# NVlabs/FoundationPose

Measured on AMD Instinct MI355X. Metric: pose-hypotheses/sec (raster+refine+score), 252 hyp x 160x160 @ 640x480 RGB-D, higher is better.
Workload: dtype f16

## Files before the change

foundationpose_amd/_lib.py:

```python
import ctypes as C
import os

import torch

_HERE = os.path.dirname(os.path.abspath(__file__))
LIB_PATH = os.environ.get("FP_AMD_LIB") or os.path.join(_HERE, "csrc", "libfp_amd.so")
ABI_VERSION = 221
_lib = None

vp, ci, cf, cd, sz = C.c_void_p, C.c_int, C.c_float, C.c_double, C.c_size_t

SIGNATURES = {
    "fp_last_error": (C.c_char_p, []),
    "fp_version": (ci, []),
    "fp_mesh_create": (ci, [vp, vp, vp, vp, vp, vp, vp, ci, ci, ci, ci, C.POINTER(vp)]),
    "fp_mesh_destroy": (None, [vp]),
    "fp_mesh_set_create": (ci, [vp, ci, C.POINTER(vp)]),
    "fp_mesh_set_destroy": (None, [vp]),
    "fp_mesh_set_workspace_bytes": (sz, [vp, ci, ci, ci]),
    "fp_depth_erode": (ci, [vp, vp, ci, ci, ci, cf, cf, cf, vp]),
    "fp_depth_bilateral": (ci, [vp, vp, ci, ci, ci, cf, cf, cf, vp]),
    "fp_depth_to_xyz": (ci, [vp, vp, cf, ci, vp, ci, ci, vp]),
    "fp_crop_windows": (ci, [vp, vp, cd, cd, ci, ci, ci, vp, vp, vp]),
    "fp_crop_windows_multi": (ci, [vp, vp, vp, vp, ci, cd, ci, ci, ci, vp, vp, vp]),
# ... 75 lines not shown
```

foundationpose_amd/csrc/conv_sw.hip:

```cpp
#include <hip/hip_fp16.h>
#include <stdlib.h>
#include <string.h>
#include <type_traits>
#include "igemm_common.h"
#include "igemm_epilogue.h"

#ifdef FP_PROFILE_BUILD
__device__ unsigned long long sw_dbg[8];
extern "C" int fp_dbg_conv_sw(unsigned long long* out, int reset) {
  if (reset) { unsigned long long z[8] = {0, 0, 0, 0, 0, 0, ~0ull, 0}; return (int)hipMemcpyToSymbol(HIP_SYMBOL(sw_dbg), z, sizeof(z)); }
  return (int)hipMemcpyFromSymbol(out, HIP_SYMBOL(sw_dbg), 8 * sizeof(unsigned long long));
}
extern "C" int fp_dbg_conv_sw_epilogue(unsigned long long* out, int reset) {
  if (reset) { unsigned long long z[8] = {0, 0, 0, 0, 0, 0, 0, 0}; return (int)hipMemcpyToSymbol(HIP_SYMBOL(ig_epi_dbg), z, sizeof(z)); }
  return (int)hipMemcpyFromSymbol(out, HIP_SYMBOL(ig_epi_dbg), 8 * sizeof(unsigned long long));
}
#define SW_CLK(t) const unsigned long long t = wall_clock64()
#else
#define SW_CLK(t)
#endif

#ifndef SW_DEFAULT_VARIANT
#define SW_DEFAULT_VARIANT 0
#endif
// ... 5 lines not shown

template <int N>
__device__ __forceinline__ void sw_wait_vm() {
  static_assert(N >= 0 && N < 64, "vmcnt is a 6-bit field");
  asm volatile("s_waitcnt vmcnt(%0)" ::"n"(N) : "memory");
}

__device__ __forceinline__ int sw_q(const IgemmGeom& g, int m) {
  const int b = ig_fastdiv(m, g.mulP, g.shrP);
  const int r = m - b * g.HoWo;
  const int oy = ig_fastdiv(r, g.mulW, g.shrW);
  const int ox = r - oy * g.Wo;
  return (b * g.Hp + oy) * g.Wp + ox;
}

template <int BM, int BN, int TM>
__global__ __launch_bounds__(512, 1) void k_conv_sw(IgemmParams p) {
  constexpr int BK = SW_BK, NW = 8, THREADS = 512;
  constexpr int NWN = BN / 64;
  static_assert((BM / (32 * TM)) * NWN == NW, "8 waves");
  constexpr int ROWB = BK * 2;
  constexpr int W_BYTES = BN * ROWB;
  constexpr int SW_PROWS = sw_prows(BM);
  constexpr int SW_PATCH_BYTES = SW_PROWS * ROWB;
  constexpr int WI = BN / 16 / NW;
  constexpr int PI = SW_PROWS / 16 / NW;
  static_assert(WI >= 1 && PI >= 1 && PI <= 7 && SW_PROWS == PI * 16 * NW, "tile shape");
  constexpr int STAGES_BYTES = 2 * SW_PATCH_BYTES + SW_NSTW * W_BYTES;
  constexpr int LDS_MAIN = ig_lds_main<BM, BN>(STAGES_BYTES);
  auto swz = [](int row) { return (row >> 2) & 3; };
  extern __shared__ __attribute__((aligned(16))) unsigned char smem[];
  SW_CLK(t_start);
  unsigned char* const patch = smem;
  unsigned char* const wring = smem + 2 * SW_PATCH_BYTES;
  const int tid = threadIdx.x, lane = tid & 63;
  const int wid = __builtin_amdgcn_readfirstlane(tid >> 6);
  const int grp = wid >> 2;
  const int wm = wid / NWN, wn = wid - wm * NWN;
  float* bias_lds = reinterpret_cast<float*>(smem + LDS_MAIN);

  const int tiles_n = p.N / BN;
  const int nwg = gridDim.x;
  const int xcd = blockIdx.x & 7, loc = blockIdx.x >> 3;
  const int qd8 = nwg >> 3, r8 = nwg & 7;
  const int tile = (xcd < r8 ? xcd * (qd8 + 1) : r8 * (qd8 + 1) + (xcd - r8) * qd8) + loc;
  const int bm = tile / tiles_n, bn = tile - bm * tiles_n;
  const int m0 = bm * BM, n0 = bn * BN;
  const int Cin = p.Cin, Ktot = 9 * Cin, Wp = p.in.Wp;
  const int ncc = Cin / BK;
  ig_bias_to_lds(p, n0, bias_lds, wid, lane);

  const int q0 = sw_q(p.in, m0);
  const int qmax = (p.M / p.in.HoWo) * p.in.Hp * Wp - 1;
  unsigned poff32[PI], woff32[WI];
#pragma unroll
  for (int j = 0; j < PI; ++j) {
    const int row = (wid * PI + j) * 16 + (lane >> 2);
    const int c = (lane & 3) ^ swz(row);
    int q = q0 + row;
    q = q < qmax ? q : qmax;
    poff32[j] = (unsigned)(((long long)q * p.in.cstride + p.in.coff + c * 8) * 2);
  }
#pragma unroll
  for (int j = 0; j < WI; ++j) {
    const int row = (wid * WI + j) * 16 + (lane >> 2);
    const int c = (lane & 3) ^ swz(row);
    woff32[j] = (unsigned)((((size_t)(n0 + row) * Ktot) + c * 8) * 2);
  }
  const bool wpk = (BN == 128) && p.Wpk != nullptr;
  if (wpk) {
#pragma unroll
    for (int j = 0; j < WI; ++j) woff32[j] = (unsigned)(((wid * WI + j) * 64 + lane) * 16);
  }
// ... 3 lines not shown

  auto stage_patch = [&](int cc, int j) {
    unsigned char* dst = patch + (cc & 1) * SW_PATCH_BYTES + (wid * PI + j) * 1024;
    __builtin_amdgcn_raw_ptr_buffer_load_lds(rsA, (__attribute__((address_space(3))) void*)dst, 16, (int)poff32[j],
                                             cc * (BK * 2), 0, 0);
  };
  auto stage_w = [&](int cc, int tap, int slot) {
    const int wsoff = wpk ? wpk_base + (cc * 9 + tap) * W_BYTES : (tap * Cin + cc * BK) * 2;
    unsigned char* dst = wring + slot * W_BYTES + wid * (WI * 1024);
#pragma unroll
    for (int j = 0; j < WI; ++j)
      __builtin_amdgcn_raw_ptr_buffer_load_lds(rsW, (__attribute__((address_space(3))) void*)(dst + j * 1024), 16,
                                               (int)woff32[j], wsoff, 0, 0);
  };

  float16_ acc[2][TM];
#pragma unroll
  for (int i = 0; i < 2; ++i)
#pragma unroll
    for (int j = 0; j < TM; ++j)
#pragma unroll
      for (int e = 0; e < 16; ++e) acc[i][j][e] = 0.f;

  const int frow = lane & 31, fhalf = lane >> 5;
  int arow[TM], w_off[2][2];
#pragma unroll
  for (int t = 0; t < TM; ++t) {
    int m = m0 + wm * (32 * TM) + t * 32 + frow;
    m = m < p.M ? m : p.M - 1;
    arow[t] = sw_q(p.in, m) - q0;
  }
#pragma unroll
  for (int t = 0; t < 2; ++t) {
    const int rw = wn * 64 + t * 32 + frow;
#pragma unroll
    for (int kk = 0; kk < 2; ++kk) w_off[t][kk] = rw * ROWB + (((2 * kk + fhalf) ^ swz(rw)) << 4);
  }

#pragma unroll
  for (int j = 0; j < PI; ++j) stage_patch(0, j);
  stage_w(0, 0, 0);
  stage_w(0, 1, 1);
  stage_w(0, 2, 2);
  sw_wait_vm<2 * WI>();
  __builtin_amdgcn_s_barrier();
  SW_CLK(t_cold);
  if (grp) __builtin_amdgcn_s_barrier();

  half8 fa[2][TM], fw[2][2];
  static_assert(TM == 4, "the four fragment addresses of the next tap are computed behind the four MFMA groups of a k-step");
  int anext[TM];
#pragma unroll
  for (int t = 0; t < TM; ++t) anext[t] = (arow[t] << 6) + ((fhalf ^ swz(arow[t])) << 4);
  auto kstep = [&](int cc, auto tap_c, auto last_c) {
    constexpr int T = decltype(tap_c)::value;
    constexpr bool LAST = decltype(last_c)::value;
    constexpr int ky = T / 3, kx = T - 3 * ky;
    const int s = cc * 9 + T;
    const unsigned char* pb = patch + (cc & 1) * SW_PATCH_BYTES;
    const unsigned char* wb = wring + (s & (SW_NSTW - 1)) * W_BYTES;
    const int shift = ky * Wp + kx;
#pragma unroll
    for (int t = 0; t < TM; ++t) {
      const int a0 = anext[t];
      fa[0][t] = *reinterpret_cast<const half8*>(pb + a0);
      fa[1][t] = *reinterpret_cast<const half8*>(pb + (a0 ^ 32));
    }
    (void)shift;
#pragma unroll
    for (int kk = 0; kk < 2; ++kk)
#pragma unroll
      for (int t = 0; t < 2; ++t) fw[kk][t] = *reinterpret_cast<const half8*>(wb + w_off[t][kk]);
    if constexpr (!LAST) {
      if constexpr (T < PI) stage_patch(cc + 1, T);
      if constexpr (T + 3 < 9) stage_w(cc, T + 3, (s + 3) & (SW_NSTW - 1));
      else stage_w(cc + 1, T - 6, (s + 3) & (SW_NSTW - 1));
      constexpr int NP = (T < PI ? 1 : 0) + ((T >= 1 && T - 1 < PI) ? 1 : 0);
      sw_wait_vm<2 * WI + NP>();
    } else {
      if constexpr (T + 3 < 9) stage_w(cc, T + 3, (s + 3) & (SW_NSTW - 1));
      constexpr int NYOUNGER = T <= 5 ? 2 : (T == 6 ? 1 : 0);
      sw_wait_vm<NYOUNGER * WI>();
    }
    asm volatile("s_waitcnt lgkmcnt(0)" ::: "memory");
    __builtin_amdgcn_sched_barrier(0);
    __builtin_amdgcn_s_barrier();
    __builtin_amdgcn_sched_barrier(0);
    __builtin_amdgcn_s_setprio(1);
    {
      constexpr int TN = (T + 1) % 9, kyn = TN / 3, kxn = TN - 3 * kyn;
      const int shift_n = kyn * Wp + kxn;
#pragma unroll
      for (int kk = 0; kk < 2; ++kk)
#pragma unroll
        for (int i = 0; i < 2; ++i) {
#pragma unroll
          for (int j = 0; j < TM; ++j)
            acc[i][j] = __builtin_amdgcn_mfma_f32_32x32x16_f16(fw[kk][i], fa[kk][j], acc[i][j], 0, 0, 0);
          const int t = kk * 2 + i;
          {
            int ar = arow[t];
            asm volatile("" : "+v"(ar));
            const int pr = ar + shift_n;
            anext[t] = (pr << 6) + ((fhalf ^ swz(pr)) << 4);
          }
        }
    }
    __builtin_amdgcn_s_setprio(0);
    __builtin_amdgcn_sched_barrier(0);
    __builtin_amdgcn_s_barrier();
    __builtin_amdgcn_sched_barrier(0);
  };
  auto chunk = [&](int cc, auto last_c) {
    kstep(cc, std::integral_constant<int, 0>{}, last_c);
    kstep(cc, std::integral_constant<int, 1>{}, last_c);
    kstep(cc, std::integral_constant<int, 2>{}, last_c);
    kstep(cc, std::integral_constant<int, 3>{}, last_c);
    kstep(cc, std::integral_constant<int, 4>{}, last_c);
    kstep(cc, std::integral_constant<int, 5>{}, last_c);
    kstep(cc, std::integral_constant<int, 6>{}, last_c);
    kstep(cc, std::integral_constant<int, 7>{}, last_c);
// ... 181 lines not shown
  ig_epilogue<BM, BN, TM, THREADS, 0>(p, acc, smem, m0, n0, wm, wn, tid, lane, bias_lds);
}

template <int BM, int BN, int TM>
int sw_ls_launch(const IgemmParams& p, hipStream_t stream) {
  constexpr int LDS = 2 * LS_PROWS * SW_BK * 2 + LS_NSTW * BN * SW_BK * 2;
  static_assert(2 * LDS <= 160 * 1024, "two workgroups per CU");
  const long long tiles = (long long)fp_cdiv(p.M, BM) * (p.N / BN);
  FP_REQUIRE(tiles < (1ll << 31), "fp_igemm_f16_fwd: too many tiles");
  FP_SET_MAX_LDS((k_conv_sw_ls<BM, BN, TM>), LDS);
  hipLaunchKernelGGL((k_conv_sw_ls<BM, BN, TM>), dim3((unsigned)tiles), dim3(256), LDS, stream, p);
  FP_CHECK_LAUNCH("fp_igemm_f16_fwd(conv_sw_ls)");
  return FP_OK;
}

template <int BM, int BN, int TM>
int sw_launch(const IgemmParams& p, hipStream_t stream) {
  constexpr int LDS = ig_lds_main<BM, BN>(2 * sw_prows(BM) * SW_BK * 2 + SW_NSTW * BN * SW_BK * 2) + IG_BIAS_LDS;
  static_assert(LDS <= 160 * 1024, "does not fit the 160 KiB LDS");
  const long long tiles = (long long)fp_cdiv(p.M, BM) * (p.N / BN);
  FP_REQUIRE(tiles < (1ll << 31), "fp_igemm_f16_fwd: too many tiles");
  FP_SET_MAX_LDS((k_conv_sw<BM, BN, TM>), LDS);
  hipLaunchKernelGGL((k_conv_sw<BM, BN, TM>), dim3((unsigned)tiles), dim3(512), LDS, stream, p);
  FP_CHECK_LAUNCH("fp_igemm_f16_fwd(conv_sw)");
  return FP_OK;
}

}

static int sw_span(const IgemmGeom& g, int BM) {
  const int row_cross = (BM - 1) / g.Wo + 1, img_cross = (BM - 1) / g.HoWo + 1;
  return (BM - 1) + 2 * row_cross + (2 * g.Wp + 2) * img_cross + 2 * g.Wp + 3;
}

static int sw_variant(const IgemmParams& p) {
  int v = SW_DEFAULT_VARIANT;
#ifdef FP_PROFILE_BUILD
  static int forced = -2;
// ... 19 lines not shown
  const IgemmGeom& g = p.in;
  if (p.taps != 9 || g.stride != 1 || g.off != 0 || g.bsplit != 0) return false;
  if (g.HoWo % g.Wo != 0 || g.Wp != g.Wo + 2 || g.Hp != g.HoWo / g.Wo + 2) return false;
  const int BM = sw_tile_rows(p);
  if (p.M % g.HoWo != 0 || p.M < 2 * BM) return false;
  if (p.Cin % 64 != 0 || p.N % 128 != 0) return false;
  const long long bytes = (long long)(p.M / g.HoWo) * g.Hp * g.Wp * g.cstride * 2;
  if (bytes >= (1ll << 31)) return false;
  return sw_span(g, BM) <= (sw_variant(p) == 1 ? LS_PROWS : sw_prows(BM));
}

int fp_conv3x3_sw_tile_rows(const IgemmParams& p) { return sw_tile_rows(p); }

int fp_conv3x3_sw_launch(const IgemmParams& p, hipStream_t stream) {
  if (sw_variant(p) == 1) return sw_ls_launch<256, 128, 4>(p, stream);
  if (sw_use_256(p)) return sw_launch<256, 256, 4>(p, stream);
  return sw_launch<512, 128, 4>(p, stream);
}

__global__ __launch_bounds__(256) void k_pack_conv3x3_tiles(const _Float16* __restrict__ w, _Float16* __restrict__ out, int N, int Cin) {
  const int nk = 9 * (Cin / 32);
  const long long total = (long long)N * nk * 4;
  const long long q = (long long)blockIdx.x * 256 + threadIdx.x;
  if (q >= total) return;
  const int pc = (int)(q & 3);
  const int r = (int)((q >> 2) & 127);
  const long long blk = q >> 9;
  const int s = (int)(blk % nk), bn = (int)(blk / nk);
  const int cc = s / 9, tap = s - 9 * cc;
  const int lc = pc ^ ((r >> 2) & 3);
  const half8 v = *reinterpret_cast<const half8*>(w + (size_t)(bn * 128 + r) * (9 * Cin) + tap * Cin + cc * 32 + lc * 8);
  *reinterpret_cast<half8*>(out + q * 8) = v;
// ... 13 lines not shown
```

foundationpose_amd/csrc/igemm.hip:

```cpp
#include <hip/hip_fp16.h>
#include <stdlib.h>
#include <string.h>
#include "igemm_common.h"
#include "igemm_epilogue.h"

int fp_igemm_pp_launch(const IgemmParams& p, int variant, hipStream_t stream);
int fp_conv3x3_sw_launch(const IgemmParams& p, hipStream_t stream);
bool fp_conv3x3_sw_applicable(const IgemmParams& p);
int fp_conv3x3_sw_tile_rows(const IgemmParams& p);

template <int BM, int BN, int TM, int NST, int BK, bool SPLITK = false>
__global__ __launch_bounds__((BM / (32 * TM)) * (BN / 64) * 64, ((BM / (32 * TM)) * (BN / 64) == 4 && TM == 4) ? 2 : 1) void k_igemm_f16(IgemmParams p) {
  constexpr int NWN = BN / 64;
  constexpr int NW = (BM / (32 * TM)) * NWN;
  constexpr int THREADS = NW * 64;
  constexpr int ROWB = BK * 2;
  constexpr int CPK = BK / 8;
  constexpr int RPI = 1024 / ROWB;
  constexpr int KK = BK / 16;
  constexpr int A_BYTES = BM * ROWB;
  constexpr int STAGE_BYTES = A_BYTES + BN * ROWB;
  constexpr int AI = BM / RPI / NW;
  constexpr int WI = BN / RPI / NW;
  static_assert(AI >= 1 && WI >= 1, "tile too small for this wave count");
// ... 295 lines not shown
  return ig_launch<128, 128, 2, 2, 64>(p, stream);
}


static int ig_build_params(const void* x, const fp_igemm_geom* x_geom, const void* w, void* y, const fp_igemm_geom* y_geom,
                           int M, int N, int Cin, int taps, const fp_igemm_epilogue* ep, IgemmParams& p, const char* who) {
  FP_REQUIRE(x && w && y && x_geom && y_geom, "%s: NULL tensor / geometry", who);
  FP_REQUIRE(taps == 1 || taps == 9, "%s: taps must be 1 (GEMM) or 9 (3x3 conv), got %d", who, taps);
  FP_REQUIRE(N > 0 && N % 128 == 0, "%s: N=%d must be a multiple of 128", who, N);
  FP_REQUIRE(Cin > 0 && Cin % 64 == 0, "%s: Cin=%d must be a multiple of 64", who, Cin);
  static const fp_igemm_epilogue no_epilogue = {nullptr, nullptr, nullptr, nullptr, nullptr, 0, nullptr, 0, nullptr, nullptr};
  const fp_igemm_epilogue& e = ep ? *ep : no_epilogue;
  FP_REQUIRE(!e.residual || e.r_geom, "%s: residual without geometry", who);
  FP_REQUIRE((e.bn_scale == nullptr) == (e.bn_shift == nullptr), "%s: bn_scale and bn_shift go together", who);
  FP_REQUIRE(!e.bn_scale || (e.flags & FP_IGEMM_ROUND_ACC), "%s: BatchNorm needs FP_IGEMM_ROUND_ACC (conv semantics)", who);
  FP_REQUIRE((e.flags & ~(FP_IGEMM_RELU | FP_IGEMM_ROUND_ACC | FP_IGEMM_HAS_W_TILES)) == 0, "%s: unknown flags 0x%x", who, e.flags);
  FP_REQUIRE((e.pe == nullptr) == (e.y_pe == nullptr) && (!e.pe || e.pe_period > 0), "%s: pe, pe_period and y_pe go together", who);
  FP_REQUIRE((((size_t)x | (size_t)w | (size_t)y | (size_t)e.residual | (size_t)e.bias | (size_t)e.bn_scale | (size_t)e.bn_shift |
               (size_t)e.pe | (size_t)e.y_pe) & 15) == 0, "%s: tensors must be 16-byte aligned", who);
  if (int err = ig_check_geom(x_geom, "input", who)) return err;
  if (int err = ig_check_geom(y_geom, "output", who)) return err;
  if (e.residual) if (int err = ig_check_geom(e.r_geom, "residual", who)) return err;
  const void* w_tiles = (e.flags & FP_IGEMM_HAS_W_TILES) ? e.w_tiles : nullptr;
  FP_REQUIRE(!w_tiles || (taps == 9 && (((size_t)w_tiles) & 15) == 0 && w_tiles != w), "%s: w_tiles is for 3x3 convolutions, 16-byte aligned, not w itself", who);
  p.A = (const _Float16*)x; p.Wt = (const _Float16*)w; p.Wpk = (const _Float16*)w_tiles; p.bias = e.bias; p.bn_scale = e.bn_scale; p.bn_shift = e.bn_shift;
  p.R = (const _Float16*)e.residual; p.Y = (_Float16*)y;
  p.pe = e.pe; p.Ype = (_Float16*)e.y_pe; p.pe_period = e.pe_period;
  p.M = M; p.N = N; p.Cin = Cin; p.taps = taps; p.relu = (e.flags & FP_IGEMM_RELU) ? 1 : 0;
  p.round_acc = (e.flags & FP_IGEMM_ROUND_ACC) ? 1 : 0;
  p.in = ig_geom(x_geom); p.out = ig_geom(y_geom); p.res = e.residual ? ig_geom(e.r_geom) : ig_geom(y_geom);
  p.slab = nullptr; p.nsplit = 0;
  return FP_OK;
}

extern "C" int fp_igemm_f16_fwd(const void* x, const fp_igemm_geom* x_geom, const void* w, void* y, const fp_igemm_geom* y_geom,
                                int M, int N, int Cin, int taps, const fp_igemm_epilogue* ep, void* stream) {
  FP_REQUIRE(M >= 0, "fp_igemm_f16_fwd: M < 0");
  if (M == 0) return FP_OK;
  IgemmParams p;
  if (int err = ig_build_params(x, x_geom, w, y, y_geom, M, N, Cin, taps, ep, p, "fp_igemm_f16_fwd")) return err;
  return ig_dispatch(p, (hipStream_t)stream);
}

extern "C" size_t fp_igemm_splitk_workspace_bytes(int M, int N, int splits) {
// ... 23 lines not shown
```

foundationpose_amd/csrc/igemm_common.h:

```cpp
#pragma once
#include <hip/hip_fp16.h>
#include "fp_common.h"

typedef _Float16 half8 __attribute__((ext_vector_type(8)));
typedef _Float16 half4 __attribute__((ext_vector_type(4)));
typedef float float16_ __attribute__((ext_vector_type(16)));

#define IG_BK 64

struct IgemmGeom {
  int HoWo, Wo;
  int Hp, Wp;
  int stride;
  int off;
  int cstride;
  int coff;
  int bsplit;
  int cgroup;
  unsigned mulP, shrP;
  unsigned mulW, shrW;
  unsigned mulB, shrB;
};

static inline void ig_fastdiv_init(int d, unsigned* mul, unsigned* shr) {
// ... 12 lines not shown
  const _Float16* A;
  const _Float16* Wt;
  const _Float16* Wpk;
  const float* bias;
  const float* bn_scale;
  const float* bn_shift;
  const _Float16* R;
  _Float16* Y;
  const float* pe;
  _Float16* Ype;
  int pe_period;
  int M, N, Cin, taps;
  int relu;
  int round_acc;
  IgemmGeom in, out, res;
  float* slab;
  int nsplit;
};

__device__ __forceinline__ long long ig_row_off(const IgemmGeom& g, int m) {
  const int b = ig_fastdiv(m, g.mulP, g.shrP);
  const int r = m - b * g.HoWo;
  const int oy = ig_fastdiv(r, g.mulW, g.shrW);
  const int ox = r - oy * g.Wo;
  int bb = b, cg = 0;
  if (g.bsplit > 0) { cg = ig_fastdiv(b, g.mulB, g.shrB); bb = b - cg * g.bsplit; }
  return (((long long)bb * g.Hp + (oy * g.stride + g.off)) * g.Wp + (ox * g.stride + g.off)) * g.cstride + g.coff +
         (long long)cg * g.cgroup;
}

// ... 1 lines not shown
```

foundationpose_amd/csrc/igemm_epilogue.h:

```cpp
#pragma once
#include "igemm_common.h"

#ifdef FP_PROFILE_BUILD
static __device__ unsigned long long ig_epi_dbg[8];
#define IG_CLK(t) const unsigned long long t = wall_clock64()
#else
#define IG_CLK(t)
#endif

#define IG_VEC_FLOATS 256
#define IG_BIAS_LDS (3 * IG_VEC_FLOATS * 4)

template <int BM, int BN>
constexpr int ig_lds_main(int stage_bytes) {
  return stage_bytes > BM * BN * 2 + BM * 16 ? stage_bytes : BM * BN * 2 + BM * 16;
}

template <int BM, int BN, int TM, int THREADS, int DBG, bool FULL>
__device__ __forceinline__ void ig_epilogue_body(const IgemmParams& p, float16_ (&acc)[2][TM], unsigned char* smem, int m0, int n0,
                                                 int wm, int wn, int tid, int lane, const float* bias_lds) {
  constexpr int CPR = BN / 8;
  constexpr int NIT = (BM * CPR) / THREADS;
  unsigned char* E = smem;
  typedef float float4_ __attribute__((ext_vector_type(4)));
  const bool round_acc = p.round_acc != 0, has_bn = p.bn_scale != nullptr;
  long long* rowY = reinterpret_cast<long long*>(smem + BM * 2 * BN);
  long long* rowR = rowY + BM;
  IG_CLK(te0);
  for (int r = tid; r < BM; r += THREADS) {
    const int m = m0 + r;
    const bool in = m < p.M;
    rowY[r] = in ? ig_row_off(p.out, m) + n0 : -1;
    if (p.R) rowR[r] = in ? ig_row_off(p.res, m) + n0 : 0;
  }
  __syncthreads();
  IG_CLK(te1);
  half8 rv[NIT];
  if (p.R) {
#pragma unroll
    for (int it = 0; it < NIT; ++it) {
      const int qd = tid + it * THREADS;
      const int ml = qd / CPR, ch = qd % CPR;
      if (FULL || rowY[ml] >= 0) rv[it] = *reinterpret_cast<const half8*>(p.R + rowR[ml] + ch * 8);
    }
  }
  IG_CLK(te2);
#pragma unroll
  for (int i = 0; i < 2; ++i) {
#pragma unroll
    for (int g = 0; g < 4; ++g) {
      const int nl = wn * 64 + i * 32 + 8 * g + 4 * (lane >> 5);
      const float4_ bv = *reinterpret_cast<const float4_*>(bias_lds + nl);
      float4_ sc = {1.f, 1.f, 1.f, 1.f}, sh = {0.f, 0.f, 0.f, 0.f};
      if (has_bn) {
        sc = *reinterpret_cast<const float4_*>(bias_lds + IG_VEC_FLOATS + nl);
        sh = *reinterpret_cast<const float4_*>(bias_lds + 2 * IG_VEC_FLOATS + nl);
      }
#pragma unroll
      for (int j = 0; j < TM; ++j) {
        const int ml = wm * (32 * TM) + j * 32 + (lane & 31);
        half4 v;
        if (round_acc) {
          typedef _Float16 half2_ __attribute__((ext_vector_type(2)));
          const half2_ b01 = {(_Float16)bv[0], (_Float16)bv[1]}, b23 = {(_Float16)bv[2], (_Float16)bv[3]};
          half2_ t01 = {(_Float16)acc[i][j][g * 4 + 0], (_Float16)acc[i][j][g * 4 + 1]};
          half2_ t23 = {(_Float16)acc[i][j][g * 4 + 2], (_Float16)acc[i][j][g * 4 + 3]};
          t01 = t01 + b01;
          t23 = t23 + b23;
          if (has_bn) {
            v[0] = (_Float16)fmaf((float)t01[0], sc[0], sh[0]);
            v[1] = (_Float16)fmaf((float)t01[1], sc[1], sh[1]);
            v[2] = (_Float16)fmaf((float)t23[0], sc[2], sh[2]);
            v[3] = (_Float16)fmaf((float)t23[1], sc[3], sh[3]);
          } else {
            v[0] = t01[0]; v[1] = t01[1]; v[2] = t23[0]; v[3] = t23[1];
          }
        } else {
#pragma unroll
          for (int e = 0; e < 4; ++e) v[e] = (_Float16)(acc[i][j][g * 4 + e] + bv[e]);
        }
        const int chunk = (nl >> 3) ^ (ml & 15);
        *reinterpret_cast<half4*>(E + ml * (2 * BN) + (chunk << 4) + ((nl & 4) << 1)) = v;
      }
    }
  }
  __syncthreads();
  IG_CLK(te3);
  const half8 zero = {0, 0, 0, 0, 0, 0, 0, 0};
#pragma unroll
  for (int it = 0; it < NIT; ++it) {
    const int qd = tid + it * THREADS;
    const int ml = qd / CPR, ch = qd % CPR;
    const long long yo = rowY[ml];
    if (!FULL && yo < 0) continue;
    half8 v = *reinterpret_cast<const half8*>(E + ml * (2 * BN) + ((ch ^ (ml & 15)) << 4));
    if (p.R) v = v + rv[it];
    if (p.relu) v = __builtin_elementwise_max(v, zero);
// ... 5 lines not shown
      half8 w;
#pragma unroll
      for (int e = 0; e < 4; ++e) { w[e] = (_Float16)((float)v[e] + e0[e]); w[4 + e] = (_Float16)((float)v[4 + e] + e1[e]); }
      *reinterpret_cast<half8*>(p.Ype + (size_t)m * p.N + n0 + ch * 8) = w;
    }
  }
#ifdef FP_PROFILE_BUILD
  IG_CLK(te4);
  if (tid == 0) {
    atomicAdd(&ig_epi_dbg[0], te1 - te0); atomicAdd(&ig_epi_dbg[1], te2 - te1); atomicAdd(&ig_epi_dbg[2], te3 - te2);
    atomicAdd(&ig_epi_dbg[3], te4 - te3); atomicAdd(&ig_epi_dbg[4], 1ull);
  }
#endif
}

template <int BM, int BN, int TM, int THREADS, int DBG = 0>
__device__ __forceinline__ void ig_epilogue(const IgemmParams& p, float16_ (&acc)[2][TM], unsigned char* smem, int m0, int n0,
                                            int wm, int wn, int tid, int lane, const float* bias_lds) {
  if (m0 + BM <= p.M) ig_epilogue_body<BM, BN, TM, THREADS, DBG, true>(p, acc, smem, m0, n0, wm, wn, tid, lane, bias_lds);
  else ig_epilogue_body<BM, BN, TM, THREADS, DBG, false>(p, acc, smem, m0, n0, wm, wn, tid, lane, bias_lds);
}
__device__ __forceinline__ void ig_bias_to_lds(const IgemmParams& p, int n0, float* bias_lds, int wid, int lane) {
  if (wid > 2) return;
  const float* src = wid == 0 ? p.bias : (wid == 1 ? p.bn_scale : p.bn_shift);
  float* dst = bias_lds + wid * IG_VEC_FLOATS;
  if (src) {
    const __amdgpu_buffer_rsrc_t rs = __builtin_amdgcn_make_buffer_rsrc(const_cast<float*>(src), 0, p.N * 4, 0x00020000);
    __builtin_amdgcn_raw_ptr_buffer_load_lds(rs, (__attribute__((address_space(3))) void*)dst, 16, lane * 16, n0 * 4, 0, 0);
  } else if (wid == 0) {
    typedef float f4 __attribute__((ext_vector_type(4)));
    *reinterpret_cast<f4*>(dst + lane * 4) = f4{0.f, 0.f, 0.f, 0.f};
  }
// ... 2 lines not shown
```

foundationpose_amd/engine.py:

```python
import contextlib

import torch
import torch.nn.functional as F

from . import ops

USE_MIOPEN = False


FUSED_OUT_PROJ_LN = True


FUSED_FFN = True


ROWS_QKV = True
ROWS_QKV_MIN_ROWS = 4096
PACKED_CONV_TILES = True
MERGED_HEAD_QKV = True
FUSED_TAIL = True


def _conv_backend():
    if USE_MIOPEN or not torch.backends.cudnn.is_available():
        return contextlib.nullcontext()
    return torch.backends.cudnn.flags(enabled=False)


def _bn_affine(sd, bn_p):
    if bn_p is None or (bn_p + ".weight") not in sd:
        return None, None
    scale = sd[bn_p + ".weight"].float() / torch.sqrt(sd[bn_p + ".running_var"].float() + 1e-5)
    shift = sd[bn_p + ".bias"].float() - sd[bn_p + ".running_mean"].float() * scale
    return scale.contiguous(), shift.contiguous()

# ... 92 lines not shown
    w = sd[conv_p + ".weight"].float()
    b = sd.get(conv_p + ".bias")
    scale, shift = _bn_affine(sd, bn_p)
    wk = w.permute(0, 2, 3, 1).reshape(w.shape[0], -1).to(torch.float16).contiguous()
    tiles = None
    if wk.is_cuda and w.shape[2] == 3 and w.shape[3] == 3 and w.shape[0] % 128 == 0 and w.shape[1] % 32 == 0 and PACKED_CONV_TILES:
        tiles = ops.pack_conv3x3_tiles(wk, w.shape[0], w.shape[1])
    return dict(w=wk, w_tiles=tiles, bias=None if b is None else _r16(b.float()), scale=scale, shift=shift)


SPLITK_MAX_HYPS = 12
HEADS_TWO_STREAMS_MAX_HYPS = 12
SPLITK_TARGET_WGS = 384
SMALL_CALL_CEILING = 31

_SWITCHES = ("FUSED_OUT_PROJ_LN", "FUSED_FFN", "ROWS_QKV", "PACKED_CONV_TILES", "MERGED_HEAD_QKV", "FUSED_TAIL", "SPLITK_MAX_HYPS", "HEADS_TWO_STREAMS_MAX_HYPS")


@contextlib.contextmanager
def overrides(**kw):
    g = globals()
    for k, v in kw.items():
        if k not in _SWITCHES:
            raise KeyError(f"engine.overrides: unknown switch {k!r} (known: {', '.join(_SWITCHES)})")
        if k.endswith("_MAX_HYPS") and not (0 <= int(v) <= SMALL_CALL_CEILING):
            raise ValueError(f"engine.overrides: {k} = {v} is outside 0..{SMALL_CALL_CEILING}")
    saved = {k: g[k] for k in kw}
    g.update(kw)
    try:
        yield
    finally:
# ... 375 lines not shown
```

foundationpose_amd/ops.py:

```python
import ctypes as C
from typing import NamedTuple

import numpy as np
import torch

from . import _lib

FLAG_NORMALIZE_XYZ = 1
FLAG_OUT_F16 = 2
MODE_REFINE = 0
MODE_SCORE = 1
ROT_AXIS_ANGLE = 0
ROT_6D = 1
TRANS_TRACKNET, TRANS_DEEPIM, TRANS_RAW = 0, 1, 2


def _stream(t=None):
    if t is None:
        return C.c_void_p(torch.cuda.current_stream().cuda_stream)
    dev = t.device
    if dev.index is not None and dev.index != torch.cuda.current_device():
        raise _lib.FpAmdError(f"tensor on {dev} but the current device is cuda:{torch.cuda.current_device()}: wrap the call in "
                              f"`with torch.cuda.device({dev.index}):` (kernels launch on the current device)")
    return C.c_void_p(torch.cuda.current_stream(dev).cuda_stream)
# ... 911 lines not shown
                                       "coff", "bsplit", "cgroup")]

    @staticmethod
    def matrix(ld):
        return IgemmGeom(1, 1, 1, 1, 1, 0, int(ld), 0, 0, 0)

    @staticmethod
    def image(Ho, Wo, pad, C_, stride=1, offset=None, coff=0, bsplit=0, cgroup=0):
        return IgemmGeom(Ho * Wo, Wo, Ho * stride + 2 * pad, Wo * stride + 2 * pad, stride, pad if offset is None else offset,
                         C_, coff, bsplit, cgroup)


IGEMM_RELU = 1
IGEMM_ROUND_ACC = 2
IGEMM_HAS_W_TILES = 4


class IgemmEpilogue(C.Structure):
    _fields_ = [("bias", C.c_void_p), ("bn_scale", C.c_void_p), ("bn_shift", C.c_void_p), ("residual", C.c_void_p),
                ("r_geom", C.POINTER(IgemmGeom)), ("flags", C.c_int), ("pe", C.c_void_p), ("pe_period", C.c_int), ("y_pe", C.c_void_p),
                ("w_tiles", C.c_void_p)]


def pack_conv3x3_tiles(w, N, Cin):
    w = _dev(w, torch.float16, "w")
    out = torch.empty_like(w)
    _lib.check(_lib.lib().fp_pack_conv3x3_tiles_f16(_ptr(w), _ptr(out), int(N), int(Cin), _stream(w)), "fp_pack_conv3x3_tiles_f16")
    return out


def igemm_f16(x, x_geom, w, bias, y, y_geom, M, N, Cin, taps, relu=False, residual=None, r_geom=None, bn_scale=None,
              bn_shift=None, conv_rounding=False, pe=None, y_pe=None, w_tiles=None):
    x = _dev(x, torch.float16, "x"); w = _dev(w, torch.float16, "w"); y = _dev(y, torch.float16, "y")
    b = _dev(bias, torch.float32, "bias"); r = _dev(residual, torch.float16, "residual")
    sc = _dev(bn_scale, torch.float32, "bn_scale"); sh = _dev(bn_shift, torch.float32, "bn_shift")
    pe = _dev(pe, torch.float32, "pe"); y_pe = _dev(y_pe, torch.float16, "y_pe")
    ep = IgemmEpilogue()
    ep.bias, ep.bn_scale, ep.bn_shift = _ptr(b), _ptr(sc), _ptr(sh)
    ep.residual = _ptr(r)
    ep.r_geom = C.pointer(r_geom) if r_geom is not None else None
    ep.flags = (IGEMM_RELU if relu else 0) | (IGEMM_ROUND_ACC if conv_rounding else 0) | IGEMM_HAS_W_TILES
    ep.pe, ep.pe_period, ep.y_pe = _ptr(pe), (int(pe.shape[-2]) if pe is not None else 0), _ptr(y_pe)
    ep.w_tiles = _ptr(_dev(w_tiles, torch.float16, "w_tiles"))
    st = _lib.lib().fp_igemm_f16_fwd(_ptr(x), C.byref(x_geom), _ptr(w), _ptr(y), C.byref(y_geom), int(M), int(N), int(Cin),
                                     int(taps), C.byref(ep), _stream(x))
    _lib.check(st, "fp_igemm_f16_fwd")
    return y


def igemm_splitk_workspace_bytes(M, N, splits):
    return int(_lib.lib().fp_igemm_splitk_workspace_bytes(int(M), int(N), int(splits)))


def igemm_f16_splitk(x, x_geom, w, bias, y, y_geom, M, N, Cin, taps, splits, workspace, relu=False, residual=None, r_geom=None,
                     bn_scale=None, bn_shift=None, conv_rounding=False, pe=None, y_pe=None):
    x = _dev(x, torch.float16, "x"); w = _dev(w, torch.float16, "w"); y = _dev(y, torch.float16, "y")
# ... 439 lines not shown
```

include/fp_amd.h:

```cpp
#ifndef FP_AMD_H
#define FP_AMD_H

#include <stddef.h>
#include <stdint.h>

#ifdef __cplusplus
extern "C" {
#endif

typedef enum {
  FP_OK = 0,
  FP_ERR_INVALID_ARG = -1,
  FP_ERR_WORKSPACE = -2,
  FP_ERR_LAUNCH = -3,
  FP_ERR_UNSUPPORTED = -4
} fp_status;

#define FP_FLAG_NORMALIZE_XYZ 1
#define FP_FLAG_OUT_F16 2

#define FP_MODE_REFINE 0
#define FP_MODE_SCORE 1

#define FP_ROT_AXIS_ANGLE 0
#define FP_ROT_6D 1
#define FP_TRANS_TRACKNET 0
#define FP_TRANS_DEEPIM 1
#define FP_TRANS_RAW 2

#define FP_SUBPIXEL_BITS 4
#define FP_ZBUF_STEPS_PER_METRE 1048576
#define FP_ZBUF_EMPTY 0xFFFFFFFFu

typedef struct fp_mesh fp_mesh;
typedef struct fp_mesh_set fp_mesh_set;

const char* fp_last_error(void);
#define FP_AMD_ABI_VERSION 221
int fp_version(void);

int fp_mesh_create(const float* pos , const float* nrm , const int32_t* faces ,
                   const float* uv , const int32_t* uv_idx ,
                   const float* tex , const float* vcol , int V, int T, int Ht,
                   int Wt, fp_mesh** out);
void fp_mesh_destroy(fp_mesh* mesh);

#define FP_MESH_SET_MAX_ELEMS (1 << 26)
int fp_mesh_set_create(const fp_mesh* const* meshes , int M, fp_mesh_set** out);
void fp_mesh_set_destroy(fp_mesh_set* set);
size_t fp_mesh_set_workspace_bytes(const fp_mesh_set* set, int N, int oh, int ow);

int fp_depth_erode(const float* depth , float* out , int H, int W, int radius,
                   float depth_diff_thres, float ratio_thres, float zfar, void* stream);
// ... 108 lines not shown
                         float input_w, void* stream);


int fp_conv7x7s2_bn_relu_fwd(const void* x , const void* w , const float* bias ,
                             const float* bn_scale , const float* bn_shift , void* y ,
                             int B, int Hin, int Win, int pad, void* stream);

typedef struct {
  int pixels_per_image, width, padded_h, padded_w, stride, offset, cstride, coff, bsplit, cgroup;
} fp_igemm_geom;

#define FP_IGEMM_RELU 1
#define FP_IGEMM_HAS_W_TILES 4
#define FP_IGEMM_ROUND_ACC 2

typedef struct {
  const float* bias;
  const float* bn_scale;
  const float* bn_shift;
  const void* residual;
  const fp_igemm_geom* r_geom;
  int flags;
  const float* pe;
  int pe_period;
  void* y_pe;
  const void* w_tiles;
} fp_igemm_epilogue;

int fp_igemm_f16_fwd(const void* x , const fp_igemm_geom* x_geom , const void* w , void* y ,
                     const fp_igemm_geom* y_geom , int M, int N, int Cin, int taps,
// ... 74 lines not shown
```

Baseline: 7489.

## Add 16x16x32 MFMA variant of the sliding-window 3x3 conv kernel

Adds a templated S16 path to the sliding-window conv kernel that uses 16x16x32 f16 MFMA instructions instead of 32x32x16. This changes fragment layout, LDS swizzle, accumulator shape and the epilogue mapping. It is selected by a new igemm flag and enabled by default from Python. The intent is to use an MFMA shape with different latency and throughput and a different LDS access pattern. The cost is more fragment loads and address arithmetic per k-step, and a new swizzle and epilogue layout that must be exactly right.

```diff
diff --git a/foundationpose_amd/_lib.py b/foundationpose_amd/_lib.py
--- a/foundationpose_amd/_lib.py
+++ b/foundationpose_amd/_lib.py
@@ -5,7 +5,7 @@
 
 _HERE = os.path.dirname(os.path.abspath(__file__))
 LIB_PATH = os.environ.get("FP_AMD_LIB") or os.path.join(_HERE, "csrc", "libfp_amd.so")
-ABI_VERSION = 221
+ABI_VERSION = 222
 _lib = None
 
 vp, ci, cf, cd, sz = C.c_void_p, C.c_int, C.c_float, C.c_double, C.c_size_t
diff --git a/foundationpose_amd/csrc/conv_sw.hip b/foundationpose_amd/csrc/conv_sw.hip
--- a/foundationpose_amd/csrc/conv_sw.hip
+++ b/foundationpose_amd/csrc/conv_sw.hip
@@ -43,7 +43,7 @@
   return (b * g.Hp + oy) * g.Wp + ox;
 }
 
-template <int BM, int BN, int TM>
+template <int BM, int BN, int TM, bool S16>
 __global__ __launch_bounds__(512, 1) void k_conv_sw(IgemmParams p) {
   constexpr int BK = SW_BK, NW = 8, THREADS = 512;
   constexpr int NWN = BN / 64;
@@ -58,6 +58,7 @@
   constexpr int STAGES_BYTES = 2 * SW_PATCH_BYTES + SW_NSTW * W_BYTES;
   constexpr int LDS_MAIN = ig_lds_main<BM, BN>(STAGES_BYTES);
   auto swz = [](int row) { return (row >> 2) & 3; };
+  auto swzp = [](int row) { return S16 ? (row >> 1) & 2 : (row >> 2) & 3; };
   extern __shared__ __attribute__((aligned(16))) unsigned char smem[];
   SW_CLK(t_start);
   unsigned char* const patch = smem;
@@ -85,7 +86,7 @@
 #pragma unroll
   for (int j = 0; j < PI; ++j) {
     const int row = (wid * PI + j) * 16 + (lane >> 2);
-    const int c = (lane & 3) ^ swz(row);
+    const int c = (lane & 3) ^ swzp(row);
     int q = q0 + row;
     q = q < qmax ? q : qmax;
     poff32[j] = (unsigned)(((long long)q * p.in.cstride + p.in.coff + c * 8) * 2);
@@ -119,27 +120,41 @@
                                                (int)woff32[j], wsoff, 0, 0);
   };
 
-  float16_ acc[2][TM];
-#pragma unroll
-  for (int i = 0; i < 2; ++i)
-#pragma unroll
-    for (int j = 0; j < TM; ++j)
-#pragma unroll
-      for (int e = 0; e < 16; ++e) acc[i][j][e] = 0.f;
-
-  const int frow = lane & 31, fhalf = lane >> 5;
-  int arow[TM], w_off[2][2];
-#pragma unroll
-  for (int t = 0; t < TM; ++t) {
-    int m = m0 + wm * (32 * TM) + t * 32 + frow;
+  constexpr int NFA = S16 ? 2 * TM : TM, NFW = S16 ? 4 : 2;
+  constexpr int FR = S16 ? 16 : 32;
+  typedef float float4_ __attribute__((ext_vector_type(4)));
+  typedef typename std::conditional<S16, float4_, float16_>::type acc_t;
+  acc_t acc[NFW][NFA];
+#pragma unroll
+  for (int i = 0; i < NFW; ++i)
+#pragma unroll
+    for (int j = 0; j < NFA; ++j)
+#pragma unroll
+      for (int e = 0; e < (S16 ? 4 : 16); ++e) acc[i][j][e] = 0.f;
+
+  const int frow = lane & (FR - 1), fhalf = lane >> (S16 ? 4 : 5);
+  int arow[NFA], w_off[2][2];
+#pragma unroll
+  for (int t = 0; t < NFA; ++t) {
+    int m = m0 + wm * (32 * TM) + t * FR + frow;
     m = m < p.M ? m : p.M - 1;
     arow[t] = sw_q(p.in, m) - q0;
-  }
-#pragma unroll
-  for (int t = 0; t < 2; ++t) {
-    const int rw = wn * 64 + t * 32 + frow;
-#pragma unroll
-    for (int kk = 0; kk < 2; ++kk) w_off[t][kk] = rw * ROWB + (((2 * kk + fhalf) ^ swz(rw)) << 4);
+    if constexpr (S16) arow[t] = (arow[t] << 6) + (fhalf << 4);
+  }
+  if constexpr (S16) {
+    const int quad = (0x1320 >> (4 * (frow >> 2))) & 3;
+#pragma unroll
+    for (int t = 0; t < 4; ++t) {
+      const int rw = wn * 64 + t * 16 + 4 * quad + (frow & 3);
+      w_off[t >> 1][t & 1] = rw * ROWB + ((fhalf ^ swz(rw)) << 4);
+    }
+  } else {
+#pragma unroll
+    for (int t = 0; t < 2; ++t) {
+      const int rw = wn * 64 + t * 32 + frow;
+#pragma unroll
+      for (int kk = 0; kk < 2; ++kk) w_off[t][kk] = rw * ROWB + (((2 * kk + fhalf) ^ swz(rw)) << 4);
+    }
   }
 
 #pragma unroll
@@ -153,10 +168,11 @@
   if (grp) __builtin_amdgcn_s_barrier();
 
   half8 fa[2][TM], fw[2][2];
-  static_assert(TM == 4, "the four fragment addresses of the next tap are computed behind the four MFMA groups of a k-step");
-  int anext[TM];
-#pragma unroll
-  for (int t = 0; t < TM; ++t) anext[t] = (arow[t] << 6) + ((fhalf ^ swz(arow[t])) << 4);
+  static_assert(TM == 4, "the fragment addresses of the next tap are computed behind the MFMA groups of a k-step, one per group of four");
+  int anext[NFA];
+#pragma unroll
+  for (int t = 0; t < NFA; ++t)
+    anext[t] = S16 ? arow[t] ^ ((arow[t] >> 3) & 32) : (arow[t] << 6) + ((fhalf ^ swz(arow[t])) << 4);
   auto kstep = [&](int cc, auto tap_c, auto last_c) {
     constexpr int T = decltype(tap_c)::value;
     constexpr bool LAST = decltype(last_c)::value;
@@ -165,17 +181,24 @@
     const unsigned char* pb = patch + (cc & 1) * SW_PATCH_BYTES;
     const unsigned char* wb = wring + (s & (SW_NSTW - 1)) * W_BYTES;
     const int shift = ky * Wp + kx;
-#pragma unroll
-    for (int t = 0; t < TM; ++t) {
-      const int a0 = anext[t];
-      fa[0][t] = *reinterpret_cast<const half8*>(pb + a0);
-      fa[1][t] = *reinterpret_cast<const half8*>(pb + (a0 ^ 32));
+    if constexpr (S16) {
+#pragma unroll
+      for (int t = 0; t < NFA; ++t) fa[t >> 2][t & 3] = *reinterpret_cast<const half8*>(pb + anext[t]);
+#pragma unroll
+      for (int t = 0; t < 4; ++t) fw[t >> 1][t & 1] = *reinterpret_cast<const half8*>(wb + w_off[t >> 1][t & 1]);
+    } else {
+#pragma unroll
+      for (int t = 0; t < TM; ++t) {
+        const int a0 = anext[t];
+        fa[0][t] = *reinterpret_cast<const half8*>(pb + a0);
+        fa[1][t] = *reinterpret_cast<const half8*>(pb + (a0 ^ 32));
+      }
+#pragma unroll
+      for (int kk = 0; kk < 2; ++kk)
+#pragma unroll
+        for (int t = 0; t < 2; ++t) fw[kk][t] = *reinterpret_cast<const half8*>(wb + w_off[t][kk]);
     }
     (void)shift;
-#pragma unroll
-    for (int kk = 0; kk < 2; ++kk)
-#pragma unroll
-      for (int t = 0; t < 2; ++t) fw[kk][t] = *reinterpret_cast<const half8*>(wb + w_off[t][kk]);
     if constexpr (!LAST) {
       if constexpr (T < PI) stage_patch(cc + 1, T);
       if constexpr (T + 3 < 9) stage_w(cc, T + 3, (s + 3) & (SW_NSTW - 1));
@@ -195,6 +218,21 @@
     {
       constexpr int TN = (T + 1) % 9, kyn = TN / 3, kxn = TN - 3 * kyn;
       const int shift_n = kyn * Wp + kxn;
+      if constexpr (S16) {
+        int sh = shift_n << 6;
+        asm volatile("" : "+s"(sh));
+#pragma unroll
+        for (int i = 0; i < 4; ++i)
+#pragma unroll
+          for (int jh = 0; jh < 2; ++jh) {
+#pragma unroll
+            for (int j = 0; j < 4; ++j)
+              acc[i][jh * 4 + j] = __builtin_amdgcn_mfma_f32_16x16x32_f16(fw[i >> 1][i & 1], fa[jh][j], acc[i][jh * 4 + j], 0, 0, 0);
+            const int t = i * 2 + jh;
+            const int x = arow[t] + sh;
+            anext[t] = x ^ ((x >> 3) & 32);
+          }
+      } else {
 #pragma unroll
       for (int kk = 0; kk < 2; ++kk)
 #pragma unroll
@@ -210,6 +248,7 @@
             anext[t] = (pr << 6) + ((fhalf ^ swz(pr)) << 4);
           }
         }
+      }
     }
     __builtin_amdgcn_s_setprio(0);
     __builtin_amdgcn_sched_barrier(0);
@@ -421,14 +460,14 @@
   return FP_OK;
 }
 
-template <int BM, int BN, int TM>
+template <int BM, int BN, int TM, bool S16>
 int sw_launch(const IgemmParams& p, hipStream_t stream) {
   constexpr int LDS = ig_lds_main<BM, BN>(2 * sw_prows(BM) * SW_BK * 2 + SW_NSTW * BN * SW_BK * 2) + IG_BIAS_LDS;
   static_assert(LDS <= 160 * 1024, "does not fit the 160 KiB LDS");
   const long long tiles = (long long)fp_cdiv(p.M, BM) * (p.N / BN);
   FP_REQUIRE(tiles < (1ll << 31), "fp_igemm_f16_fwd: too many tiles");
-  FP_SET_MAX_LDS((k_conv_sw<BM, BN, TM>), LDS);
-  hipLaunchKernelGGL((k_conv_sw<BM, BN, TM>), dim3((unsigned)tiles), dim3(512), LDS, stream, p);
+  FP_SET_MAX_LDS((k_conv_sw<BM, BN, TM, S16>), LDS);
+  hipLaunchKernelGGL((k_conv_sw<BM, BN, TM, S16>), dim3((unsigned)tiles), dim3(512), LDS, stream, p);
   FP_CHECK_LAUNCH("fp_igemm_f16_fwd(conv_sw)");
   return FP_OK;
 }
@@ -478,8 +517,8 @@
 
 int fp_conv3x3_sw_launch(const IgemmParams& p, hipStream_t stream) {
   if (sw_variant(p) == 1) return sw_ls_launch<256, 128, 4>(p, stream);
-  if (sw_use_256(p)) return sw_launch<256, 256, 4>(p, stream);
-  return sw_launch<512, 128, 4>(p, stream);
+  if (sw_use_256(p)) return p.mfma16 ? sw_launch<256, 256, 4, true>(p, stream) : sw_launch<256, 256, 4, false>(p, stream);
+  return p.mfma16 ? sw_launch<512, 128, 4, true>(p, stream) : sw_launch<512, 128, 4, false>(p, stream);
 }
 
 __global__ __launch_bounds__(256) void k_pack_conv3x3_tiles(const _Float16* __restrict__ w, _Float16* __restrict__ out, int N, int Cin) {
diff --git a/foundationpose_amd/csrc/igemm.hip b/foundationpose_amd/csrc/igemm.hip
--- a/foundationpose_amd/csrc/igemm.hip
+++ b/foundationpose_amd/csrc/igemm.hip
@@ -333,7 +333,10 @@
   FP_REQUIRE(!e.residual || e.r_geom, "%s: residual without geometry", who);
   FP_REQUIRE((e.bn_scale == nullptr) == (e.bn_shift == nullptr), "%s: bn_scale and bn_shift go together", who);
   FP_REQUIRE(!e.bn_scale || (e.flags & FP_IGEMM_ROUND_ACC), "%s: BatchNorm needs FP_IGEMM_ROUND_ACC (conv semantics)", who);
-  FP_REQUIRE((e.flags & ~(FP_IGEMM_RELU | FP_IGEMM_ROUND_ACC | FP_IGEMM_HAS_W_TILES)) == 0, "%s: unknown flags 0x%x", who, e.flags);
+  FP_REQUIRE((e.flags & ~(FP_IGEMM_RELU | FP_IGEMM_ROUND_ACC | FP_IGEMM_HAS_W_TILES | FP_IGEMM_MFMA_16X16X32 | FP_IGEMM_MFMA_32X32X16)) == 0,
+             "%s: unknown flags 0x%x", who, e.flags);
+  FP_REQUIRE((e.flags & (FP_IGEMM_MFMA_16X16X32 | FP_IGEMM_MFMA_32X32X16)) != (FP_IGEMM_MFMA_16X16X32 | FP_IGEMM_MFMA_32X32X16),
+             "%s: FP_IGEMM_MFMA_16X16X32 and FP_IGEMM_MFMA_32X32X16 exclude each other", who);
   FP_REQUIRE((e.pe == nullptr) == (e.y_pe == nullptr) && (!e.pe || e.pe_period > 0), "%s: pe, pe_period and y_pe go together", who);
   FP_REQUIRE((((size_t)x | (size_t)w | (size_t)y | (size_t)e.residual | (size_t)e.bias | (size_t)e.bn_scale | (size_t)e.bn_shift |
                (size_t)e.pe | (size_t)e.y_pe) & 15) == 0, "%s: tensors must be 16-byte aligned", who);
@@ -347,6 +350,7 @@
   p.pe = e.pe; p.Ype = (_Float16*)e.y_pe; p.pe_period = e.pe_period;
   p.M = M; p.N = N; p.Cin = Cin; p.taps = taps; p.relu = (e.flags & FP_IGEMM_RELU) ? 1 : 0;
   p.round_acc = (e.flags & FP_IGEMM_ROUND_ACC) ? 1 : 0;
+  p.mfma16 = (e.flags & FP_IGEMM_MFMA_32X32X16) ? 0 : ((e.flags & FP_IGEMM_MFMA_16X16X32) ? 1 : SW_DEFAULT_MFMA16);
   p.in = ig_geom(x_geom); p.out = ig_geom(y_geom); p.res = e.residual ? ig_geom(e.r_geom) : ig_geom(y_geom);
   p.slab = nullptr; p.nsplit = 0;
   return FP_OK;
diff --git a/foundationpose_amd/csrc/igemm_common.h b/foundationpose_amd/csrc/igemm_common.h
--- a/foundationpose_amd/csrc/igemm_common.h
+++ b/foundationpose_amd/csrc/igemm_common.h
@@ -7,6 +7,9 @@
 typedef float float16_ __attribute__((ext_vector_type(16)));
 
 #define IG_BK 64
+#ifndef SW_DEFAULT_MFMA16
+#define SW_DEFAULT_MFMA16 1
+#endif
 
 struct IgemmGeom {
   int HoWo, Wo;
@@ -50,6 +53,7 @@
   int relu;
   int round_acc;
   IgemmGeom in, out, res;
+  int mfma16;
   float* slab;
   int nsplit;
 };
diff --git a/foundationpose_amd/csrc/igemm_epilogue.h b/foundationpose_amd/csrc/igemm_epilogue.h
--- a/foundationpose_amd/csrc/igemm_epilogue.h
+++ b/foundationpose_amd/csrc/igemm_epilogue.h
@@ -1,4 +1,5 @@
 #pragma once
+#include <type_traits>
 #include "igemm_common.h"
 
 #ifdef FP_PROFILE_BUILD
@@ -16,9 +17,12 @@
   return stage_bytes > BM * BN * 2 + BM * 16 ? stage_bytes : BM * BN * 2 + BM * 16;
 }
 
-template <int BM, int BN, int TM, int THREADS, int DBG, bool FULL>
-__device__ __forceinline__ void ig_epilogue_body(const IgemmParams& p, float16_ (&acc)[2][TM], unsigned char* smem, int m0, int n0,
+typedef float ig_float4 __attribute__((ext_vector_type(4)));
+template <int BM, int BN, int TM, int THREADS, int DBG, bool FULL, typename Acc>
+__device__ __forceinline__ void ig_epilogue_body(const IgemmParams& p, Acc& acc, unsigned char* smem, int m0, int n0,
                                                  int wm, int wn, int tid, int lane, const float* bias_lds) {
+  constexpr bool S16 = std::is_same<Acc, ig_float4[4][2 * TM]>::value;
+  static_assert(S16 || std::is_same<Acc, float16_[2][TM]>::value, "accumulator layout");
   constexpr int CPR = BN / 8;
   constexpr int NIT = (BM * CPR) / THREADS;
   unsigned char* E = smem;
@@ -45,42 +49,63 @@
     }
   }
   IG_CLK(te2);
+  auto put4 = [&](int nl, int ml, float a0, float a1, float a2, float a3, const float4_& bv, const float4_& sc, const float4_& sh) {
+    half4 v;
+    if (round_acc) {
+      typedef _Float16 half2_ __attribute__((ext_vector_type(2)));
+      const half2_ b01 = {(_Float16)bv[0], (_Float16)bv[1]}, b23 = {(_Float16)bv[2], (_Float16)bv[3]};
+      half2_ t01 = {(_Float16)a0, (_Float16)a1};
+      half2_ t23 = {(_Float16)a2, (_Float16)a3};
+      t01 = t01 + b01;
+      t23 = t23 + b23;
+      if (has_bn) {
+        v[0] = (_Float16)fmaf((float)t01[0], sc[0], sh[0]);
+        v[1] = (_Float16)fmaf((float)t01[1], sc[1], sh[1]);
+        v[2] = (_Float16)fmaf((float)t23[0], sc[2], sh[2]);
+        v[3] = (_Float16)fmaf((float)t23[1], sc[3], sh[3]);
+      } else {
+        v[0] = t01[0]; v[1] = t01[1]; v[2] = t23[0]; v[3] = t23[1];
+      }
+    } else {
+      v[0] = (_Float16)(a0 + bv[0]); v[1] = (_Float16)(a1 + bv[1]); v[2] = (_Float16)(a2 + bv[2]); v[3] = (_Float16)(a3 + bv[3]);
+    }
+    const int chunk = (nl >> 3) ^ (ml & 15);
+    *reinterpret_cast<half4*>(E + ml * (2 * BN) + (chunk << 4) + ((nl & 4) << 1)) = v;
+  };
+  auto vecs = [&](int nl, float4_& bv, float4_& sc, float4_& sh) {
+    bv = *reinterpret_cast<const float4_*>(bias_lds + nl);
+    sc = float4_{1.f, 1.f, 1.f, 1.f}; sh = float4_{0.f, 0.f, 0.f, 0.f};
+    if (has_bn) {
+      sc = *reinterpret_cast<const float4_*>(bias_lds + IG_VEC_FLOATS + nl);
+      sh = *reinterpret_cast<const float4_*>(bias_lds + 2 * IG_VEC_FLOATS + nl);
+    }
+  };
+  if constexpr (S16) {
+    const int quad = (0x1320 >> (4 * (lane >> 4))) & 3;
 #pragma unroll
-  for (int i = 0; i < 2; ++i) {
+    for (int i = 0; i < 4; ++i) {
+      const int nl = wn * 64 + i * 16 + 4 * quad;
+      float4_ bv, sc, sh;
+      vecs(nl, bv, sc, sh);
 #pragma unroll
-    for (int g = 0; g < 4; ++g) {
-      const int nl = wn * 64 + i * 32 + 8 * g + 4 * (lane >> 5);
-      const float4_ bv = *reinterpret_cast<const float4_*>(bias_lds + nl);
-      float4_ sc = {1.f, 1.f, 1.f, 1.f}, sh = {0.f, 0.f, 0.f, 0.f};
-      if (has_bn) {
-        sc = *reinterpret_cast<const float4_*>(bias_lds + IG_VEC_FLOATS + nl);
-        sh = *reinterpret_cast<const float4_*>(bias_lds + 2 * IG_VEC_FLOATS + nl);
+      for (int j = 0; j < 2 * TM; ++j) {
+        const int ml = wm * (32 * TM) + j * 16 + (lane & 15);
+        put4(nl, ml, acc[i][j][0], acc[i][j][1], acc[i][j][2], acc[i][j][3], bv, sc, sh);
       }
+    }
+  } else {
 #pragma unroll
-      for (int j = 0; j < TM; ++j) {
-        const int ml = wm * (32 * TM) + j * 32 + (lane & 31);
-        half4 v;
-        if (round_acc) {
-          typedef _Float16 half2_ __attribute__((ext_vector_type(2)));
-          const half2_ b01 = {(_Float16)bv[0], (_Float16)bv[1]}, b23 = {(_Float16)bv[2], (_Float16)bv[3]};
-          half2_ t01 = {(_Float16)acc[i][j][g * 4 + 0], (_Float16)acc[i][j][g * 4 + 1]};
-          half2_ t23 = {(_Float16)acc[i][j][g * 4 + 2], (_Float16)acc[i][j][g * 4 + 3]};
-          t01 = t01 + b01;
-          t23 = t23 + b23;
-          if (has_bn) {
-            v[0] = (_Float16)fmaf((float)t01[0], sc[0], sh[0]);
-            v[1] = (_Float16)fmaf((float)t01[1], sc[1], sh[1]);
-            v[2] = (_Float16)fmaf((float)t23[0], sc[2], sh[2]);
-            v[3] = (_Float16)fmaf((float)t23[1], sc[3], sh[3]);
-          } else {
-            v[0] = t01[0]; v[1] = t01[1]; v[2] = t23[0]; v[3] = t23[1];
-          }
-        } else {
+    for (int i = 0; i < 2; ++i) {
 #pragma unroll
-          for (int e = 0; e < 4; ++e) v[e] = (_Float16)(acc[i][j][g * 4 + e] + bv[e]);
+      for (int g = 0; g < 4; ++g) {
+        const int nl = wn * 64 + i * 32 + 8 * g + 4 * (lane >> 5);
+        float4_ bv, sc, sh;
+        vecs(nl, bv, sc, sh);
+#pragma unroll
+        for (int j = 0; j < TM; ++j) {
+          const int ml = wm * (32 * TM) + j * 32 + (lane & 31);
+          put4(nl, ml, acc[i][j][g * 4 + 0], acc[i][j][g * 4 + 1], acc[i][j][g * 4 + 2], acc[i][j][g * 4 + 3], bv, sc, sh);
         }
-        const int chunk = (nl >> 3) ^ (ml & 15);
-        *reinterpret_cast<half4*>(E + ml * (2 * BN) + (chunk << 4) + ((nl & 4) << 1)) = v;
       }
     }
   }
@@ -116,8 +141,8 @@
 #endif
 }
 
-template <int BM, int BN, int TM, int THREADS, int DBG = 0>
-__device__ __forceinline__ void ig_epilogue(const IgemmParams& p, float16_ (&acc)[2][TM], unsigned char* smem, int m0, int n0,
+template <int BM, int BN, int TM, int THREADS, int DBG = 0, typename Acc>
+__device__ __forceinline__ void ig_epilogue(const IgemmParams& p, Acc& acc, unsigned char* smem, int m0, int n0,
                                             int wm, int wn, int tid, int lane, const float* bias_lds) {
   if (m0 + BM <= p.M) ig_epilogue_body<BM, BN, TM, THREADS, DBG, true>(p, acc, smem, m0, n0, wm, wn, tid, lane, bias_lds);
   else ig_epilogue_body<BM, BN, TM, THREADS, DBG, false>(p, acc, smem, m0, n0, wm, wn, tid, lane, bias_lds);
diff --git a/foundationpose_amd/engine.py b/foundationpose_amd/engine.py
--- a/foundationpose_amd/engine.py
+++ b/foundationpose_amd/engine.py
@@ -19,6 +19,7 @@
 PACKED_CONV_TILES = True
 MERGED_HEAD_QKV = True
 FUSED_TAIL = True
+CONV_MFMA_16X16X32 = True
 
 
 def _conv_backend():
@@ -141,7 +142,7 @@
 SPLITK_TARGET_WGS = 384
 SMALL_CALL_CEILING = 31
 
-_SWITCHES = ("FUSED_OUT_PROJ_LN", "FUSED_FFN", "ROWS_QKV", "PACKED_CONV_TILES", "MERGED_HEAD_QKV", "FUSED_TAIL", "SPLITK_MAX_HYPS", "HEADS_TWO_STREAMS_MAX_HYPS")
+_SWITCHES = ("FUSED_OUT_PROJ_LN", "FUSED_FFN", "ROWS_QKV", "PACKED_CONV_TILES", "MERGED_HEAD_QKV", "FUSED_TAIL", "CONV_MFMA_16X16X32", "SPLITK_MAX_HYPS", "HEADS_TWO_STREAMS_MAX_HYPS")
 
 
 @contextlib.contextmanager
diff --git a/foundationpose_amd/ops.py b/foundationpose_amd/ops.py
--- a/foundationpose_amd/ops.py
+++ b/foundationpose_amd/ops.py
@@ -949,6 +949,8 @@
 IGEMM_RELU = 1
 IGEMM_ROUND_ACC = 2
 IGEMM_HAS_W_TILES = 4
+IGEMM_MFMA_16X16X32 = 16
+IGEMM_MFMA_32X32X16 = 32
 
 
 class IgemmEpilogue(C.Structure):
@@ -965,7 +967,7 @@
 
 
 def igemm_f16(x, x_geom, w, bias, y, y_geom, M, N, Cin, taps, relu=False, residual=None, r_geom=None, bn_scale=None,
-              bn_shift=None, conv_rounding=False, pe=None, y_pe=None, w_tiles=None):
+              bn_shift=None, conv_rounding=False, pe=None, y_pe=None, w_tiles=None, mfma16=None):
     x = _dev(x, torch.float16, "x"); w = _dev(w, torch.float16, "w"); y = _dev(y, torch.float16, "y")
     b = _dev(bias, torch.float32, "bias"); r = _dev(residual, torch.float16, "residual")
     sc = _dev(bn_scale, torch.float32, "bn_scale"); sh = _dev(bn_shift, torch.float32, "bn_shift")
@@ -974,7 +976,11 @@
     ep.bias, ep.bn_scale, ep.bn_shift = _ptr(b), _ptr(sc), _ptr(sh)
     ep.residual = _ptr(r)
     ep.r_geom = C.pointer(r_geom) if r_geom is not None else None
-    ep.flags = (IGEMM_RELU if relu else 0) | (IGEMM_ROUND_ACC if conv_rounding else 0) | IGEMM_HAS_W_TILES
+    if mfma16 is None:
+        from . import engine
+        mfma16 = engine.CONV_MFMA_16X16X32
+    ep.flags = (IGEMM_RELU if relu else 0) | (IGEMM_ROUND_ACC if conv_rounding else 0) | IGEMM_HAS_W_TILES | \
+        (IGEMM_MFMA_16X16X32 if mfma16 else IGEMM_MFMA_32X32X16)
     ep.pe, ep.pe_period, ep.y_pe = _ptr(pe), (int(pe.shape[-2]) if pe is not None else 0), _ptr(y_pe)
     ep.w_tiles = _ptr(_dev(w_tiles, torch.float16, "w_tiles"))
     st = _lib.lib().fp_igemm_f16_fwd(_ptr(x), C.byref(x_geom), _ptr(w), _ptr(y), C.byref(y_geom), int(M), int(N), int(Cin),
diff --git a/include/fp_amd.h b/include/fp_amd.h
--- a/include/fp_amd.h
+++ b/include/fp_amd.h
@@ -36,7 +36,7 @@
 typedef struct fp_mesh_set fp_mesh_set;
 
 const char* fp_last_error(void);
-#define FP_AMD_ABI_VERSION 221
+#define FP_AMD_ABI_VERSION 222
 int fp_version(void);
 
 int fp_mesh_create(const float* pos , const float* nrm , const int32_t* faces ,
@@ -175,6 +175,9 @@
 #define FP_IGEMM_HAS_W_TILES 4
 #define FP_IGEMM_ROUND_ACC 2
 
+#define FP_IGEMM_MFMA_16X16X32 16
+#define FP_IGEMM_MFMA_32X32X16 32
+
 typedef struct {
   const float* bias;
   const float* bn_scale;
```

New measurement: 7632, median of 6. 1.02x the previous value.
